# pppKin/rs_ray_toy

Hardware: AMD Instinct MI355X
Metric: Mrays/s (BVH ray queries, closest+any) @ 100k-tri heightfield 1024^2 256spp depth 8 (higher is better)
Workload: dtype f32; 1 GPU; BASELINE cfg4: procedural heightfield 100352 triangles, 1024x1024, 256 spp, Path max_depth 8, HaltonSampler, RealisticCamera, box filter; fixed-bvh BVH; film in interleaved 16-row bands, one gather to rank 0 per frame; 2 frame(s) in flight; collective=none (one rank), comm_world=1, triangles=100352, bvh_nodes=97951, bvh_depth=24

## Files before the change

### rs_ray_toy_amd/csrc/device/dkernels.hpp

```cpp
#pragma once
#include "dmath.hpp"
#include "dtexture.hpp"

namespace rrtd {

constexpr int kBlock = 256;
enum { C_ACTIVE = 0, C_NEXT = 32, C_SHADOW = 64, C_CAMERA_RAYS = 96, C_ERROR = 128, C_WORK_CLOSEST = 160, C_WORK_SHADOW = 192, C_WORK_AUX = 224, C_SHADOW2 = 256,
       C_WORK8_CLOSEST = 288, C_WORK8_SHADOW = 544,
       C_TT_DONE = 800,
       C_CULLED = 832,
       C_SKY = 864,
       C_RECORDS = 896, C_COUNT = 928 };
template <typename R> struct ShadeBlock { static constexpr int n = 256; };
#ifndef RRT_SHADE_BLOCK
#define RRT_SHADE_BLOCK 256
#endif
template <> struct ShadeBlock<float> { static constexpr int n = RRT_SHADE_BLOCK; };
enum { ERR_SHADING_NORMAL = 1, ERR_BETA = 4, ERR_NULL_BSDF = 8, ERR_MIPMAP = 16, ERR_HALTON_DIMS = 32, ERR_ST_DIMS = 64, ERR_NO_LIGHTS = 128,
       ERR_KIND_SET = 256  };
static_assert(ERR_ST_DIMS == kErrStDims, "error bit shared with dmath.hpp");
static_assert(ERR_HALTON_DIMS == kErrHaltonDims, "error bit shared with dmath.hpp");

template <typename R>
struct RayCtx {
// ... 850 lines not shown
#define RRT_SHADE_CHUNK 4u
#endif
#ifndef RRT_SHADE_WAVES
#define RRT_SHADE_WAVES 4
#endif
#ifndef RRT_SHADE_WAVES_LAMBERT
#define RRT_SHADE_WAVES_LAMBERT 6
#endif
#ifndef RRT_SHADE_BLOCK_LAMBERT
#define RRT_SHADE_BLOCK_LAMBERT 512
#endif
#ifndef RRT_SHADE_WAVES_GLOSSY
#define RRT_SHADE_WAVES_GLOSSY RRT_SHADE_WAVES
#endif
#ifndef RRT_SHADE_BLOCK_GLOSSY
#define RRT_SHADE_BLOCK_GLOSSY RRT_SHADE_BLOCK
#endif
template <typename R, uint32_t KM> constexpr int shade_path_block() {
  return sizeof(R) != 4 ? ShadeBlock<R>::n : (KM == kKindsLambert ? RRT_SHADE_BLOCK_LAMBERT : (KM == kKindsGlossy ? RRT_SHADE_BLOCK_GLOSSY : ShadeBlock<R>::n));
}
template <uint32_t KM> constexpr int shade_path_waves() { return KM == kKindsLambert ? RRT_SHADE_WAVES_LAMBERT : (KM == kKindsGlossy ? RRT_SHADE_WAVES_GLOSSY : RRT_SHADE_WAVES); }
template <typename R, int NL, bool TEX = false, uint32_t KM = kAllKinds, bool AREA = true>
__global__ void __launch_bounds__((shade_path_block<R, KM>())) __attribute__((amdgpu_waves_per_eu(TEX ? 1 : shade_path_waves<KM>(), 8))) k_shade_path(SceneDev<R> s, Pools<R> p) {
  __shared__ uint32_t push_lds[shade_path_block<R, KM>() / 64 + 1];
  constexpr uint32_t kShadeChunk = RRT_SHADE_CHUNK;
  __shared__ uint32_t hit_idx[kShadeChunk * shade_path_block<R, KM>()];
  const uint32_t n = p.counters[C_ACTIVE];
  using V4 = typename Vec4T<R>::type;
  const uint32_t chunk = s.shade_compact ? kShadeChunk : 1u;
  for (uint32_t base0 = blockIdx.x * blockDim.x * chunk; base0 < n; base0 += gridDim.x * blockDim.x * chunk) {
  uint32_t n_hits = min(blockDim.x, n - base0);
  if (chunk > 1u) {
    n_hits = 0u;
    for (uint32_t k = 0; k < chunk; k++) {
      const uint32_t e = base0 + k * blockDim.x + threadIdx.x;
      const bool is_hit = e < n && (int)real_to_bits(p.hit[e].y) >= 0;
      uint32_t cnt = 0;
      const uint32_t at = block_rank(is_hit, push_lds, &cnt);
      if (is_hit) hit_idx[n_hits + at] = e;
      n_hits += cnt;
    }
    __syncthreads();
  }
  for (uint32_t base = 0; base < n_hits; base += blockDim.x) {
  const uint32_t i = base + threadIdx.x < n_hits ? (chunk > 1u ? hit_idx[base + threadIdx.x] : base0 + base + threadIdx.x) : n;
  bool want_shadow = false, want_next = false, sky = false;
  uint32_t slot = 0;
  int prim = -1;
  V3<R> sh_o, sh_d, nx_o, nx_d, o_lo;
  Rgb<R> sh_ld, nx_beta;
  R nx_eta_scale = R(1);
  uint32_t index = 0, nx_db = 0, sh_tab = 0;
  if (i < n) {
    const QEnt qe = p.q_active[i];
    slot = qe.slot;
// ... 68 lines not shown
          if (cont && (int)bounces < s.max_depth && s.horizon != nullptr) {
            const float u = s.hz_axis == 0u ? (float)nd.x : (s.hz_axis == 1u ? (float)nd.y : (float)nd.z);
            const float a = s.hz_axis == 0u ? (float)nd.y : (s.hz_axis == 1u ? (float)nd.z : (float)nd.x), b = s.hz_axis == 0u ? (float)nd.z : (s.hz_axis == 1u ? (float)nd.x : (float)nd.y);
            const uint32_t q = s.horizon[(size_t)prim * 32u + (u < 0.0f ? 16u : 0u) + hz_sector(a, b)];
#ifdef RRT_HZ_NO_GUARD
            const float tau = -1.0f;
#else
            const float tau = s.hz_tau[prim];
#endif
            const bool above = fabsf(u) * 254.0f > (float)q;
            const bool inside = fminf(fminf((float)h.z, (float)h.w), 1.0f - (float)h.z - (float)h.w) * fabsf((float)dot(si.n, nd)) > tau;
            if (above && inside) { cont = false; sky = true; }
          }
          if (cont && (int)bounces < s.max_depth) {
            nx_o = si.p; nx_d = nd;
            nx_beta = beta; nx_eta_scale = eta_scale;
            nx_db = db_pack(s, dim, bounces);
            want_next = true;
          }
        }
      }
    }
  }
  const uint32_t qs = block_push(p.shadow_count, want_shadow, push_lds);
  if (want_shadow) {
    store_ray<R>(p.sray_o, p.sray_d, qs, sh_o, o_lo, sh_d, R(1) - R(0.0001), self_prim<R>(prim) | (int)(sh_tab << 24));
    p.sld[qs] = mk4u<R>(sh_ld.r, sh_ld.g, sh_ld.b, slot);
  }
  const uint32_t qn = block_push(&p.counters[C_NEXT], want_next, push_lds);
  if (want_next) {
    p.q_next[qn] = QEnt{slot, nx_db, index, 0u};
    p.npath[qn] = mk4<R>(nx_beta.r, nx_beta.g, nx_beta.b, nx_eta_scale);
    store_ray<R>(p.nray_o, p.nray_d, qn, nx_o, o_lo, nx_d, Const<R>::inf, self_prim<R>(prim));
  }
  if (s.horizon != nullptr) (void)block_push(&p.counters[C_SKY], sky, push_lds);
  }
  __syncthreads();
  }
}

template <typename R>
__global__ void __launch_bounds__(ShadeBlock<R>::n) k_shade_nee(SceneDev<R> s, Pools<R> p, int light_j, int first) {
  __shared__ uint32_t push_lds[ShadeBlock<R>::n / 64 + 1];
  using V4 = typename Vec4T<R>::type;
  const uint32_t i = blockIdx.x * blockDim.x + threadIdx.x;
  const uint32_t n = p.counters[C_ACTIVE];
  if (blockIdx.x * blockDim.x >= n) return;
  bool want_shadow = false;
  uint32_t slot = 0, sh_tab = 0;
  int prim = -1;
  V3<R> sh_o, sh_d, o_lo;
  Rgb<R> sh_ld;
  if (i < n) {
    const QEnt qe = p.q_active[i];
    slot = qe.slot;
    const V4 h = p.hit[i];
    prim = (int)real_to_bits(h.y);
    if (prim >= 0) {
// ... 223 lines not shown
          } else {
            R eta = R(1) / bsdf.eta;
            if (dot(wo, ns) < R(0)) { eta = R(1) / eta; ns = -ns; dndx = -dndx; dndy = -dndy; }
            const V3<R> dwodx = -fdr.rxd - wo, dwody = -fdr.ryd - wo;
            const R ddndx = dot(dwodx, ns) + dot(wo, dndx), ddndy = dot(dwody, ns) + dot(wo, dndy);
            const R mu = eta * dot(wo, ns) - absdot(wi, ns);
            const R dmudx = ddndx * (eta - (eta * eta * dot(wo, ns)) / absdot(wi, ns));
            const R dmudy = ddndy * (eta - (eta * eta * dot(wo, ns)) / absdot(wi, ns));
            cd.rxd = wi - dwodx * eta + (dndx * mu + ns * dmudx);
            cd.ryd = wi - dwody * eta + (dndy * mu + ns * dmudy);
          }
          c.dr = cd;
        }
      }
    }
  }
  V4 l = p.L[qe.slot];
  l.x += L.r; l.y += L.g; l.z += L.b;
  p.L[qe.slot] = l;
  if (n_closest) atomicAdd(&totals[2], (unsigned long long)n_closest);
  if (n_any) atomicAdd(&totals[3], (unsigned long long)n_any);
}

static __global__ void k_rotate(uint32_t* c, int what) {
  if (what == 0) { c[C_ACTIVE] = c[C_NEXT]; c[C_NEXT] = 0; c[C_SHADOW] = 0; }
  else if (what == 1) { c[C_SHADOW] = 0; }
  else if (what == 3) {  }
  else if (what == 4) { c[C_NEXT] = 0; }
  else if (what == 5) { c[C_ACTIVE] = c[C_NEXT]; c[C_NEXT] = 0; c[C_WORK_CLOSEST] = 0; c[C_WORK_AUX] = 0; for (int k = 0; k < 8; k++) c[C_WORK8_CLOSEST + 32 * k] = 0; return; }
  else if (what == 6) { c[C_SHADOW] = 0; c[C_WORK_SHADOW] = 0; for (int k = 0; k < 8; k++) c[C_WORK8_SHADOW + 32 * k] = 0; return; }
  else if (what == 7) { c[C_SHADOW2] = 0; c[C_WORK_SHADOW] = 0; for (int k = 0; k < 8; k++) c[C_WORK8_SHADOW + 32 * k] = 0; return; }
  else { c[C_ACTIVE] = 0; c[C_NEXT] = 0; c[C_SHADOW] = 0; c[C_RECORDS] = 0; }
  c[C_WORK_CLOSEST] = 0; c[C_WORK_SHADOW] = 0; c[C_WORK_AUX] = 0;
  for (int k = 0; k < 8; k++) { c[C_WORK8_CLOSEST + 32 * k] = 0; c[C_WORK8_SHADOW + 32 * k] = 0; }
}
static __global__ void k_accumulate_counts(uint32_t* c, unsigned long long* totals) {
  totals[2] += c[C_ACTIVE];
}
static __global__ void k_accumulate_shadow(const uint32_t* shadow_count, unsigned long long* totals) { totals[3] += *shadow_count; }
static __global__ void k_accumulate_sky(uint32_t* c, unsigned long long* totals) { totals[2] += c[C_SKY]; totals[8] += c[C_SKY]; c[C_SKY] = 0; }
static __global__ void k_accumulate_camera(uint32_t* c, unsigned long long* totals) {
  totals[4] += c[C_CAMERA_RAYS]; c[C_CAMERA_RAYS] = 0;
  totals[2] += c[C_CULLED]; totals[7] += c[C_CULLED]; c[C_CULLED] = 0;
}

template <typename R>
RRT_DEV Rgb<R> film_sample_radiance(const SceneDev<R>& s, R w, const typename Vec4T<R>::type& l) {
  Rgb<R> L;
  if (w > R(0)) L = Rgb<R>(l.x, l.y, l.z);
  if (L.has_nan()) L = Rgb<R>();
  else if (L.y() < R(-1e-5)) L = Rgb<R>();
  else if (isinf(L.y())) L = Rgb<R>();
  if (L.y() > s.max_sample_luminance) L = L * (s.max_sample_luminance / L.y());
  return L;
}
template <typename R>
RRT_DEV void film_box_add(const SceneDev<R>& s, R& cr, R& cg, R& cb, R& wsum, R w, const typename Vec4T<R>::type& l) {
  const Rgb<R> L = film_sample_radiance(s, w, l);
  cr += (L.r * w) * R(1); cg += (L.g * w) * R(1); cb += (L.b * w) * R(1);
  wsum += R(1);
}

template <typename R>
// ... 375 lines not shown
```

### rs_ray_toy_amd/csrc/device/dmath.hpp

```cpp
#pragma once
#include "dtypes.hpp"

namespace rrtd {

#define RRT_DEV __device__ __forceinline__

template <typename R> struct Const;
template <> struct Const<float> {
  static constexpr float one_minus_eps = 0.99999994f;
  static constexpr float machine_eps = 5.9604645e-8f;
  static constexpr float inf = __builtin_huge_valf();
};
template <> struct Const<double> {
  static constexpr double one_minus_eps = 0.99999999999999989;
  static constexpr double machine_eps = 1.1102230246251565e-16;
  static constexpr double inf = __builtin_huge_val();
};
#define RRT_PI 3.14159265358979323846
#define RRT_PI_OVER_2 1.57079632679489661923
#define RRT_PI_OVER_4 0.78539816339744830961

template <typename R> RRT_DEV R rsqrt_(R x) { return sqrt(x); }
RRT_DEV double rcp_r(double a) { return 1.0 / a; }
RRT_DEV float rcp_r(float a) { return __builtin_amdgcn_rcpf(a); }
// ... 103 lines not shown
  const uint32_t base = lds[nw] + lds[w];
  __syncthreads();
  return base + (uint32_t)__popcll(mask & ((1ull << lane) - 1ull));
}

RRT_DEV uint32_t block_push_range(uint32_t* counter, bool pred, uint32_t* lds, uint32_t* first, uint32_t* total) {
  const uint64_t mask = __ballot(pred);
  const uint32_t lane = __lane_id(), w = threadIdx.x >> 6, nw = (blockDim.x + 63u) >> 6;
  if (lane == 0) lds[w] = (uint32_t)__popcll(mask);
  __syncthreads();
  if (threadIdx.x == 0) {
    uint32_t tot = 0;
    for (uint32_t k = 0; k < nw; k++) { const uint32_t c = lds[k]; lds[k] = tot; tot += c; }
    lds[nw] = tot ? atomicAdd(counter, tot) : 0u;
    lds[nw + 1] = tot;
  }
  __syncthreads();
  *first = lds[nw]; *total = lds[nw + 1];
  const uint32_t base = lds[nw] + lds[w];
  __syncthreads();
  return base + (uint32_t)__popcll(mask & ((1ull << lane) - 1ull));
}

template <uint32_t... kOff>
RRT_DEV void block_push_multi(uint32_t* counters, uint32_t on, uint32_t pred, uint32_t* lds, uint32_t* at, uint32_t* first, uint32_t* total) {
  constexpr uint32_t kN = sizeof...(kOff);
  constexpr uint32_t off[kN] = {kOff...};
  const uint32_t lane = __lane_id(), w = threadIdx.x >> 6, nw = (blockDim.x + 63u) >> 6, stride = nw + 2u;
  uint64_t mask[kN];
#pragma unroll
  for (uint32_t i = 0; i < kN; i++) {
    mask[i] = __ballot((pred >> i) & 1u);
    if (lane == 0) lds[i * stride + w] = (uint32_t)__popcll(mask[i]);
  }
  __syncthreads();
  if (threadIdx.x < kN) {
    uint32_t o = off[0];
#pragma unroll
    for (uint32_t i = 1; i < kN; i++) if (threadIdx.x == i) o = off[i];
    uint32_t* l = lds + threadIdx.x * stride;
    uint32_t tot = 0;
    for (uint32_t k = 0; k < nw; k++) { const uint32_t n = l[k]; l[k] = tot; tot += n; }
    l[nw] = (tot && ((on >> threadIdx.x) & 1u)) ? atomicAdd(counters + o, tot) : 0u;
    l[nw + 1] = tot;
  }
  __syncthreads();
  const uint64_t below = (1ull << lane) - 1ull;
#pragma unroll
  for (uint32_t i = 0; i < kN; i++) {
    first[i] = lds[i * stride + nw]; total[i] = lds[i * stride + nw + 1];
    at[i] = first[i] + lds[i * stride + w] + (uint32_t)__popcll(mask[i] & below);
  }
  __syncthreads();
}

RRT_DEV uint32_t block_rank(bool pred, uint32_t* lds, uint32_t* total) {
  const uint64_t mask = __ballot(pred);
  const uint32_t lane = __lane_id(), w = threadIdx.x >> 6, nw = (blockDim.x + 63u) >> 6;
  if (lane == 0) lds[w] = (uint32_t)__popcll(mask);
  __syncthreads();
  if (threadIdx.x == 0) {
    uint32_t tot = 0;
    for (uint32_t k = 0; k < nw; k++) { const uint32_t c = lds[k]; lds[k] = tot; tot += c; }
    lds[nw] = tot;
  }
  __syncthreads();
  const uint32_t base = lds[w];
  *total = lds[nw];
  __syncthreads();
  return base + (uint32_t)__popcll(mask & ((1ull << lane) - 1ull));
}

RRT_DEV uint32_t div_base(uint32_t a, const HaltonDim& hd, uint32_t ) {
  const uint32_t t = __umulhi((uint32_t)hd.magic, a);
  return (t + ((a - t) >> 1)) >> (uint32_t)(hd.magic >> 32);
}
// ... 778 lines not shown
```

### rs_ray_toy_amd/csrc/device/dtraverse_f32.hpp

```cpp
#pragma once
#include "dkernels.hpp"
#include "lens_cull.hpp"

#ifndef RRT_VOTE_A
#define RRT_VOTE_A 1u
#define RRT_VOTE_B 2u
#endif
#ifndef RRT_NODE_STEPS
#define RRT_NODE_STEPS 2
#endif
#ifndef RRT_TR_REFILL
#define RRT_TR_REFILL 16u
#endif
namespace rrtd {

constexpr int kTravBlock = 512;
constexpr int kStackLds = 8;
constexpr int kTreeletNodes = 512;

struct alignas(64) PairNode {
  float xy0[4];
  float xy1[4];
  float zz[4];
  uint32_t id0, id1;
// ... 1151 lines not shown
        if (s.integrator != 0 ) p.path[qa] = make_float4(1.0f, 1.0f, 1.0f, 1.0f);
        p.ray_o[qa] = make_float4(wo.x, wo.y, wo.z, Const<float>::inf);
        p.ray_d[qa] = make_float4(wd.x, wd.y, wd.z, __uint_as_float(0xffffffffu));
      }
      if (!runs) { p.L[slot] = make_float4(0.0f, 0.0f, 0.0f, 0.0f); p.weight[slot] = w; }
      else if (rec) p.L[ref] = make_float4(0.0f, 0.0f, 0.0f, w);
    }
  }
}

RRT_DEV bool rg_trace_lean(const SceneDev<float>& s, const RgLensLds& lens, float pfx, float pfy, float lx, float ly, bool want_ray, RayT<float>& out) {
  RgLane L; L.phase = 0;
  const float w = rg_begin_lean(s, pfx, pfy, lx, ly, &L);
  bool ok = w != 0.0f;
  for (int k = s.n_lens - 1; k >= 0; k--) ok &= rg_step_lean(lens.a[k], lens.b[k], &L);
  if (ok && want_ray) {
    out.o = aff_pt(s.cam_m, V3<float>(L.o.x, L.o.y, -L.o.z));
    const V3<float> wdu = aff_vec(s.cam_m, V3<float>(L.d.x, L.d.y, -L.d.z));
    out.d = wdu * __builtin_amdgcn_rsqf(len2(wdu));
  }
  return ok;
}

static __global__ void __launch_bounds__(kRgDense) k_raygen_aux2_f32(SceneDev<float> s, Pools<float> p, int enqueue, int records) {
  __shared__ RgLensLds lens;
  __shared__ uint32_t push_lds[kRgDense / 64 + 1];
  const uint32_t tid = threadIdx.x;
  const uint32_t n = p.counters[C_NEXT];
  if (blockIdx.x * blockDim.x >= n) return;
  rg_lens_to_lds(s, &lens, tid);
  __syncthreads();
  const uint32_t i = blockIdx.x * blockDim.x + tid;
  const bool diffs = p.rdx_o != nullptr;
  bool alive = false;
  uint32_t slot = 0;
  float4 ro = make_float4(0, 0, 0, 0), rd = ro, cs = ro;
  if (i < n) {
    ro = p.nray_o[i]; rd = p.nray_d[i];
    slot = __float_as_uint(ro.w);
    cs = p.npath[i];
  }
  RayT<float> aux, auy;
  float epsx = 0.05f, epsy = 0.05f;
  bool okx = false, oky = false;
  for (int round = 0; round < 4; round++) {
    const bool is_x = (round & 1) == 0;
    const bool act = i < n && (round < 2 || (round == 2 ? !okx : (okx && !oky)));
    if (__ballot(act) == 0ull) continue;
    const float e = round < 2 ? 0.05f : -0.05f;
    RayT<float> out;
    bool ok = false;
    if (act) ok = rg_trace_lean(s, lens, cs.x + (is_x ? e : 0.0f), cs.y + (is_x ? 0.0f : e), cs.z, cs.w, diffs, out);
    if (act && is_x) { okx = ok; epsx = e; if (diffs) aux = out; }
    if (act && !is_x) { oky = ok; epsy = e; if (diffs) auy = out; }
  }
  alive = okx && oky;
  if (i < n) {
    if (alive && diffs) {
      const V3<float> o(ro.x, ro.y, ro.z), d(rd.x, rd.y, rd.z);
      V3<float> rxo = o + (aux.o - o) / epsx, rxd = d + (aux.d - d) / epsx;
      V3<float> ryo = o + (auy.o - o) / epsy, ryd = d + (auy.d - d) / epsy;
      rxo = o + (rxo - o) * s.diff_scale; ryo = o + (ryo - o) * s.diff_scale;
      rxd = d + (rxd - d) * s.diff_scale; ryd = d + (ryd - d) * s.diff_scale;
      p.rdx_o[slot] = make_float4(rxo.x, rxo.y, rxo.z, 0.0f); p.rdx_d[slot] = make_float4(rxd.x, rxd.y, rxd.z, 0.0f);
      p.rdy_o[slot] = make_float4(ryo.x, ryo.y, ryo.z, 0.0f); p.rdy_d[slot] = make_float4(ryd.x, ryd.y, ryd.z, 0.0f);
    }
  }
  const bool meets = !(s.root_cull && alive) || camera_ray_meets_root(s, V3<float>(ro.x, ro.y, ro.z), V3<float>(rd.x, rd.y, rd.z));
  const bool enq = alive && enqueue && meets;
  const uint32_t q = block_push(&p.counters[C_ACTIVE], enq, push_lds);
  if (s.root_cull) (void)block_push(&p.counters[C_CULLED], alive && enqueue && !meets, push_lds);
  (void)block_push(&p.counters[C_CAMERA_RAYS], alive, push_lds);
  if (enq) {
    p.q_active[q] = QEnt{slot, 5u, p.hindex[i], 0u};
    if (s.integrator != 0 ) p.path[q] = make_float4(1.0f, 1.0f, 1.0f, 1.0f);
    p.ray_o[q] = make_float4(ro.x, ro.y, ro.z, Const<float>::inf);
    p.ray_d[q] = make_float4(rd.x, rd.y, rd.z, __uint_as_float(0xffffffffu));
  }
  if (records) { if (i < n) p.L[slot] = make_float4(0.0f, 0.0f, 0.0f, alive ? rd.w : 0.0f); }
  else if (alive) { p.L[slot] = make_float4(0.0f, 0.0f, 0.0f, 0.0f); p.weight[slot] = rd.w; }
}

constexpr uint32_t kFrTiles = 4;
typedef float v4f __attribute__((ext_vector_type(4)));
static __global__ void __launch_bounds__(64 * kFrTiles) k_film_box_runs(SceneDev<float> s, Pools<float> p, PassDesc pd, float* film, const uint2* runs, uint32_t n_groups) {
  __shared__ v4f tab[kFrTiles][8][64];
  const uint32_t lane = threadIdx.x & 63u, wv = threadIdx.x >> 6;
  const uint32_t tile = blockIdx.x * kFrTiles + wv;
  const bool live = tile < pd.npix / 64u;
  const uint32_t* code = reinterpret_cast<const uint32_t*>(p.weight);
  float cr = 0.0f, cg = 0.0f, cb = 0.0f, wsum = 0.0f;
  float* px = film;
  if (live) {
    uint32_t x, y;
    pass_pixel(pd, pd.pix_begin + tile * 64u + lane, &x, &y);
    px = film + 4 * ((size_t)y * (uint32_t)s.xres + x);
    cr = px[0]; cg = px[1]; cb = px[2]; wsum = px[3];
  }
#pragma unroll
  for (uint32_t k = 0; k < 8; k++) tab[wv][k][lane] = v4f{0.0f, 0.0f, 0.0f, 0.0f};
  v4f rec[2][8];
  uint32_t cd[2][8];
  auto load = [&](auto B, uint32_t first, uint32_t cnt) {
// ... 41 lines not shown
```

### rs_ray_toy_amd/csrc/device/dtypes.hpp

```cpp
#pragma once
#include <hip/hip_runtime.h>
#include <stdint.h>

#include "horizon_build.hpp"
namespace rrtd {
struct HaltonBlk {
  uint32_t block;
  uint32_t shift;
  uint32_t magic;
  uint32_t lo_off, hi_off;
  uint32_t pad[3];
};

template <typename R>
struct alignas(sizeof(R) * 8) Node {
  R bmin[3];
  R bmax[3];
  uint32_t offset;
  uint32_t meta;
};

template <typename R>
struct alignas(16) Tri {
  R p0[3], p1[3], p2[3];
// ... 110 lines not shown
  uint32_t hz_axis;
  float root_box[6];
  const LensElem<R>* lens;
  int32_t n_lens, simple_weighting;
  R cam_m[12];
  R pupil0[4], pupil63[4];
  R shutter_open, shutter_close;
  int32_t xres, yres;
  R diagonal, extent[4];
  R max_sample_luminance;
  const R* filter_table;
  R filter_rx, filter_ry;
  R filter_inv_rx, filter_inv_ry;
  const HaltonDim* hdims;
  uint32_t* err;
  const uint16_t* perms;
  uint32_t nsamp, sample_at_center;
  uint32_t base_exp0, base_exp1, base_scale0, base_scale1, stride, mult_inv0, mult_inv1;
  uint32_t fast_div;
  uint32_t sampler_type;
  uint32_t st_nx, st_ny, st_jitter, st_dims, st_seed_lo, st_seed_hi;
  uint32_t cam_db;
  uint32_t shade_compact;
  uint32_t db_shift;
  uint32_t cam_perm[2];
  double cam_invpow[2][16];
  double cam_tail[2];
  double inv_base_scale1;
  double inv3pow[24];
  const uint32_t* cam_lo[3];
  const uint4* cam_hi[3];
  const HaltonBlk* hblk;
  const uint32_t* hlo;
  const uint4* hhi;
  uint32_t n_hblk;
  int32_t integrator, max_depth, light_strategy;
  R rr_threshold;
};

template <typename R> struct Vec4T;
template <> struct Vec4T<float> { using type = float4; };
template <> struct Vec4T<double> { using type = double4; };

struct alignas(16) QEnt { uint32_t slot, db, index, pad; };

template <typename R>
// ... 21 lines not shown
```

### rs_ray_toy_amd/csrc/device/rrt_impl.hpp

```cpp
#pragma once
#include <algorithm>
#include <atomic>
#include <chrono>
#include <cmath>
#include <cstdio>
#include <cstring>
#include <deque>
#include <mutex>
#include <memory>
#include <queue>
#include <stdexcept>
#include <string>
#include <thread>
#include <unordered_map>
#include <vector>

#include <type_traits>

#include "dfilter.hpp"
#include "dkernels.hpp"
#include "dtraverse_f32.hpp"
#include "rrt.h"

namespace rrtd {
// ... 498 lines not shown
  void gather_mark(bool begin) override {
    if (!pending_ || !frame_stats_) return;
    HIP_CHECK(hipSetDevice(dev_));
    hipEvent_t& e = ev_gather_[begin ? 0 : 1];
    if (!e) HIP_CHECK(hipEventCreate(&e));
    HIP_CHECK(hipEventRecord(e, st_));
    if (!begin) gather_marked_ = true;
  }
  void film_geometry(int* xres, int* yres, bool* splats) const override {
    const rrt_film& f = desc_.film;
    *xres = f.xres; *yres = f.yres;
    *splats = f.filter_type != RRT_FILTER_BOX || f.filter_radius[0] > 0.5 || f.filter_radius[1] > 0.5;
  }

  void set_option(const std::string& key, double v) override {
    if (key == "max_paths") { if (v < 64) throw std::invalid_argument("max_paths must be >= 64"); max_paths_ = (size_t)v; }
    else if (key == "count_traversal") count_traversal_ = v != 0;
    else if (key == "persistent_traversal") { persistent_ = v != 0; if (v >= 1) trav_mode_ = (int)v; }
    else if (key == "raygen_lean") raygen_lean_ = v != 0;
    else if (key == "tile_order") tile_order_ = v != 0;
    else if (key == "tile_trees") tile_trees_on_ = v != 0;
    else if (key == "quad_nodes") quad_on_ = v != 0;
    else if (key == "shade_compact") scene_.shade_compact = v != 0 ? 1u : 0u;
    else if (key == "horizon_cull") horizon_on_ = v != 0;
    else if (key == "root_cull") root_cull_on_ = v != 0;
    else if (key == "tt_census") { tt_census_spp_ = std::max(1, (int)v); tt_state_ = 0; }
    else if (key == "shadow_lists") shadow_lists_on_ = v != 0;
    else if (key == "sl_grid") sl_grid_cap_ = std::max(1, (int)v);
    else if (key == "rg_spb") {
      if (v != 1 && v != 2 && v != 4 && v != 8) throw std::invalid_argument("rg_spb must be 1, 2, 4 or 8");
      rg_spb_ = (int)v;
    }
    else if (key == "pt_split_closest") pt_split_closest_ = (uint32_t)v;
    else if (key == "pt_split_any") pt_split_any_ = (uint32_t)v;
    else if (key == "overlap_shadow") overlap_shadow_ = v != 0;
    else if (key == "aux_margin") aux_margin_ = v != 0;
    else if (key == "lens_cull") lens_cull_on_ = v != 0;
    else if (key == "film_records") film_records_on_ = v != 0;
    else if (key == "shade_spec") shade_kinds_ = v != 0 ? shade_kinds_scene_ : kAllKinds;
    else if (key == "frame_stats") frame_stats_ = v != 0;
    else if (key == "dn_lds") dn_lds_ = v != 0;
    else if (key == "halton_tables") scene_.n_hblk = (v != 0 && hblk_.n) ? (uint32_t)kHaltonTabDims : 0u;
    else if (key == "cam_tables") { for (int w = 0; w < 3; w++) { scene_.cam_lo[w] = (v != 0 && cam_lo_.n) ? cam_lo_.p + cam_lo_off_[w] : nullptr; scene_.cam_hi[w] = (v != 0 && cam_hi_.n) ? cam_hi_.p + cam_hi_off_[w] : nullptr; } }
    else if (key == "any_entry") { any_entry_on_ = v != 0; trav_.any_list = (any_entry_on_ && any_list_.n) ? reinterpret_cast<const uint4*>(any_list_.p) : nullptr; }
    else if (key == "nonblocking_streams") {
      if (pending_) throw std::invalid_argument("nonblocking_streams: a frame is in flight");
// ... 217 lines not shown
    };
    auto tock = [&](size_t id, hipStream_t stream = nullptr) { if (timing) HIP_CHECK(hipEventRecord(evs[id].second.second, stream ? stream : st_)); };
    uint64_t& n_closest_launch = fr->n_closest_launch;
    uint64_t& n_any_launch = fr->n_any_launch;
    const int integ = desc_.integrator.type;
    const int max_depth = desc_.integrator.max_depth;
    const size_t npix = pd.npix;
    const uint64_t ns = pd.ns;
    const size_t nslots = npix * (size_t)ns;
    const uint32_t grid = (uint32_t)((nslots + kBlock - 1) / kBlock);
    const uint32_t sgrid = (uint32_t)((nslots + ShadeBlock<R>::n - 1) / ShadeBlock<R>::n);
    hipLaunchKernelGGL(k_rotate, dim3(1), dim3(1), 0, st_, counters_.p, 2);
    size_t e = tick(0);
    launch_raygen(pd, grid, nullptr, integ != RRT_INT_AO ? 1 : 0, true, !with_moments, list);
    tock(e);
    hipLaunchKernelGGL(k_accumulate_camera, dim3(1), dim3(1), 0, st_, counters_.p, totals_.p);
    if (integ == RRT_INT_PATH) {
      const bool overlap = two_shadow_queues() && shadow_buf_[1][0] && !count_traversal_ && max_depth > 1;
      auto use_shadow_queue = [&](int k) {
        pool_.sray_o = shadow_buf_[k][0]; pool_.sray_d = shadow_buf_[k][1]; pool_.sld = shadow_buf_[k][2];
        pool_.shadow_count = counters_.p + (k ? C_SHADOW2 : C_SHADOW);
      };
      for (int b = 0; b < max_depth; b++) {
        hipLaunchKernelGGL(k_accumulate_counts, dim3(1), dim3(1), 0, st_, counters_.p, totals_.p);
        e = tick(1);
        launch_closest(nullptr, &counters_.p[C_ACTIVE], 0, count_traversal_, nullptr, nullptr, count_traversal_ ? totals_.p : nullptr, grid, b == 0);
        tock(e); n_closest_launch++;
        if (b == 0 && tt_pass_ok_ && !count_traversal_ && use_persistent()) fr->n_tile_launch++;
        if (overlap) {
          use_shadow_queue(b & 1);
          if (b > 1) HIP_CHECK(hipStreamWaitEvent(st_, ev_shadow_[b & 1], 0));
        }
        scene_.use_shadow_tabs = use_shadow_lists() ? 1u : 0u;
        scene_.horizon = (horizon_on_ && horizon_.n) ? horizon_.p : nullptr; scene_.hz_tau = horizon_tau_.p; scene_.hz_axis = hz_axis_;
        e = tick(3);
        if (tex_depth_ > 0) hipLaunchKernelGGL((k_shade_path<R, 4, true>), dim3(std::min((uint32_t)((nslots + 255) / 256), 16384u)), dim3(256), 0, st_, scene_, pool_);
        else if (has_translucent_) hipLaunchKernelGGL((k_shade_path<R, 4>), dim3(std::min((uint32_t)((nslots + 255) / 256), 16384u)), dim3(256), 0, st_, scene_, pool_);
        else if (shade_kinds_ == kKindsLambert) {
          constexpr uint32_t kB = (uint32_t)shade_path_block<R, kKindsLambert>();
          const dim3 g(std::min((uint32_t)((nslots + kB - 1) / kB), 16384u));
          if (area_lights_ || shade_kinds_ == kAllKinds) hipLaunchKernelGGL((k_shade_path<R, 2, false, kKindsLambert, true>), g, dim3(kB), 0, st_, scene_, pool_);
          else hipLaunchKernelGGL((k_shade_path<R, 2, false, kKindsLambert, false>), g, dim3(kB), 0, st_, scene_, pool_);
        }
        else if (shade_kinds_ == kKindsGlossy) {
          constexpr uint32_t kB = (uint32_t)shade_path_block<R, kKindsGlossy>();
          hipLaunchKernelGGL((k_shade_path<R, 2, false, kKindsGlossy>), dim3(std::min((uint32_t)((nslots + kB - 1) / kB), 16384u)), dim3(kB), 0, st_, scene_, pool_);
        }
        else hipLaunchKernelGGL((k_shade_path<R, 2>), dim3(std::min(sgrid, 16384u)), dim3(ShadeBlock<R>::n), 0, st_, scene_, pool_);
        tock(e);
        if (scene_.horizon) hipLaunchKernelGGL(k_accumulate_sky, dim3(1), dim3(1), 0, st_, counters_.p, totals_.p);
        if (overlap) {
          HIP_CHECK(hipEventRecord(ev_shade_, st_));
          HIP_CHECK(hipStreamWaitEvent(st2_, ev_shade_, 0));
          hipLaunchKernelGGL(k_accumulate_shadow, dim3(1), dim3(1), 0, st2_, pool_.shadow_count, totals_.p);
          e = tick(2, st2_);
          launch_shadow(grid, st2_);
          tock(e, st2_); n_any_launch++; if (use_shadow_lists()) fr->n_list_launch++;
          hipLaunchKernelGGL(k_rotate, dim3(1), dim3(1), 0, st2_, counters_.p, 6 + (b & 1));
          HIP_CHECK(hipEventRecord(ev_shadow_[b & 1], st2_));
          swap_queues();
          hipLaunchKernelGGL(k_rotate, dim3(1), dim3(1), 0, st_, counters_.p, 5);
        } else {
          hipLaunchKernelGGL(k_accumulate_shadow, dim3(1), dim3(1), 0, st_, pool_.shadow_count, totals_.p);
          e = tick(2);
          launch_shadow(grid);
          tock(e); n_any_launch++; if (use_shadow_lists()) fr->n_list_launch++;
          swap_queues();
          hipLaunchKernelGGL(k_rotate, dim3(1), dim3(1), 0, st_, counters_.p, 0);
        }
      }
      if (overlap) {
        HIP_CHECK(hipStreamWaitEvent(st_, ev_shadow_[(max_depth - 1) & 1], 0));
        use_shadow_queue(0);
      }
    } else if (integ == RRT_INT_DIRECT || integ == RRT_INT_DEBUG) {
      if (has_transmissive_ || tex_depth_ > 0) {
        size_t e2 = tick(3);
        TreeFrame<R>* deep = nullptr;
        if (max_depth > kTreeMax) {
          const size_t need = (size_t)(max_depth - kTreeMax) * nslots;
          if (tree_deep_.n < need) { HIP_CHECK(hipStreamSynchronize(st_)); tree_deep_.alloc(need); }
          deep = tree_deep_.p;
        }
        if (tex_depth_ > 0) hipLaunchKernelGGL((k_direct_tree<R, true>), dim3(grid), dim3(kBlock), 0, st_, scene_, pool_, totals_.p, deep, (uint32_t)nslots);
        else hipLaunchKernelGGL((k_direct_tree<R, false>), dim3(grid), dim3(kBlock), 0, st_, scene_, pool_, totals_.p, deep, (uint32_t)nslots);
        tock(e2);
      } else {
      const bool all = integ == RRT_INT_DEBUG || desc_.integrator.light_strategy == RRT_STRATEGY_ALL;
      for (int level = 0; level < std::max(1, max_depth - 1); level++) {
        hipLaunchKernelGGL(k_accumulate_counts, dim3(1), dim3(1), 0, st_, counters_.p, totals_.p);
        e = tick(1);
        launch_closest(nullptr, &counters_.p[C_ACTIVE], 0, count_traversal_, nullptr, nullptr, count_traversal_ ? totals_.p : nullptr, grid, level == 0);
        tock(e); n_closest_launch++;
        if (level == 0 && tt_pass_ok_ && !count_traversal_ && use_persistent()) fr->n_tile_launch++;
        if (desc_.n_lights > 0) {
          const int nl = all ? (int)desc_.n_lights : 1;
          for (int j = 0; j < nl; j++) {
            hipLaunchKernelGGL(k_rotate, dim3(1), dim3(1), 0, st_, counters_.p, 1);
            scene_.use_shadow_tabs = use_shadow_lists() ? 1u : 0u;
            e = tick(3);
            hipLaunchKernelGGL((k_shade_nee<R>), dim3(sgrid), dim3(ShadeBlock<R>::n), 0, st_, scene_, pool_, all ? j : -1, j == 0 ? 1 : 0);
            tock(e);
            hipLaunchKernelGGL(k_accumulate_shadow, dim3(1), dim3(1), 0, st_, pool_.shadow_count, totals_.p);
            e = tick(2);
            launch_shadow(grid);
            tock(e); n_any_launch++; if (use_shadow_lists()) fr->n_list_launch++;
          }
        }
        e = tick(3);
        hipLaunchKernelGGL((k_shade_specular<R>), dim3(sgrid), dim3(ShadeBlock<R>::n), 0, st_, scene_, pool_, (desc_.n_lights == 0 && integ == RRT_INT_DEBUG) ? 1 : 0);
        tock(e);
        swap_queues();
        hipLaunchKernelGGL(k_rotate, dim3(1), dim3(1), 0, st_, counters_.p, 0);
      }
      }
    }
    e = tick(4);
    if (!wide_filter && film_runs_ok_) {
      if constexpr (std::is_same<R, float>::value)
        hipLaunchKernelGGL(k_film_box_runs, dim3((uint32_t)((npix / 64 + kFrTiles - 1) / kFrTiles)), dim3(64 * kFrTiles), 0, st_, scene_, pool_, pd, film_.p, film_runs_.p, (uint32_t)(ns / 8));
    }
    else if (!wide_filter) {
      const dim3 fg((uint32_t)((npix + kBlock - 1) / kBlock));
      if (list) hipLaunchKernelGGL((k_film_box_moments_list<R>), fg, dim3(kBlock), 0, st_, scene_, pool_, pd, list, film_.p, moments_.p);
      else if (with_moments) hipLaunchKernelGGL((k_film_box_moments<R>), fg, dim3(kBlock), 0, st_, scene_, pool_, pd, film_.p, moments_.p);
      else hipLaunchKernelGGL((k_film_box<R>), fg, dim3(kBlock), 0, st_, scene_, pool_, pd, film_.p);
    }
    else {
      const int reach_x = (int)std::ceil(f.filter_radius[0] + 0.5), reach_y = (int)std::ceil(f.filter_radius[1] + 0.5);
      const int ex0 = std::max(0, rect[0] - reach_x), ey0 = std::max(0, rect[1] - reach_y);
      const int ex1 = std::min(f.xres, rect[2] + reach_x), ey1 = std::min(f.yres, rect[3] + reach_y);
      const size_t en = (size_t)(ex1 - ex0) * (size_t)(ey1 - ey0);
      const dim3 fg((uint32_t)((en + kBlock - 1) / kBlock));
      if (with_moments) hipLaunchKernelGGL((k_film_wide_moments<R>), fg, dim3(kBlock), 0, st_, scene_, pool_, pd, film_.p, moments_.p, ex0, ey0, ex1 - ex0, ey1 - ey0, reach_x, reach_y, f.yres);
      else hipLaunchKernelGGL((k_film_wide<R>), fg, dim3(kBlock), 0, st_, scene_, pool_, pd, film_.p, ex0, ey0, ex1 - ex0, ey1 - ey0, reach_x, reach_y, f.yres);
    }
// ... 861 lines not shown
          }
        }
        cam_lo_.upload(lo_all, st_); cam_hi_.upload(hi_all, st_);
        HIP_CHECK(hipStreamSynchronize(st_));
        for (int w = 0; w < 3; w++) { cam_lo_off_[w] = lo_off[w]; cam_hi_off_[w] = hi_off[w]; s.cam_lo[w] = cam_lo_.p + lo_off[w]; s.cam_hi[w] = cam_hi_.p + hi_off[w]; }
      }
    }
    {
      std::vector<R> ft(256);
      for (int i = 0; i < 256; i++) ft[i] = (R)d->film.filter_table[i];
      filter_table_.upload(ft, st_);
      HIP_CHECK(hipStreamSynchronize(st_));
      s.filter_table = filter_table_.p;
      s.filter_rx = (R)d->film.filter_radius[0]; s.filter_ry = (R)d->film.filter_radius[1];
      s.filter_inv_rx = (R)(1.0 / d->film.filter_radius[0]); s.filter_inv_ry = (R)(1.0 / d->film.filter_radius[1]);
    }
    s.sampler_type = (uint32_t)d->sampler.type;
    s.st_nx = (uint32_t)std::max(1, d->sampler.xsamp); s.st_ny = (uint32_t)std::max(1, d->sampler.ysamp);
    s.st_jitter = d->sampler.jitter ? 1u : 0u; s.st_dims = (uint32_t)std::max(0, d->sampler.dimension);
    s.st_seed_lo = (uint32_t)d->sampler.perm_seed; s.st_seed_hi = (uint32_t)(d->sampler.perm_seed >> 32);
    s.cam_db = d->sampler.type == RRT_SAMPLER_STRATIFIED ? (1u | (2u << kStBits)) : 5u;
    s.db_shift = d->sampler.type == RRT_SAMPLER_STRATIFIED ? kDbShiftStratified : kDbShiftHalton;
    s.shade_compact = 1u;
    s.integrator = d->integrator.type; s.max_depth = d->integrator.max_depth; s.light_strategy = d->integrator.light_strategy;
    s.rr_threshold = (R)d->integrator.rr_threshold;
    counters_.alloc(C_COUNT);
    HIP_CHECK(hipMemsetAsync(counters_.p, 0, C_COUNT * sizeof(uint32_t), st_));
    s.err = counters_.p + C_ERROR;
  }

  bool two_shadow_queues() const { return overlap_shadow_ && desc_.integrator.type == RRT_INT_PATH && !deep_; }
  size_t n_vec_records() const { return 12 + (tex_depth_ > 0 ? 4 : 0) + (two_shadow_queues() ? 3 : 0); }
  void ensure_pools(size_t n) {
    if (n <= cap_) return;
    HIP_CHECK(hipStreamSynchronize(st_));
    cap_ = n;
    using V4 = typename Vec4T<R>::type;
    const size_t NV = n_vec_records(), NR = 1, NU = 9;
    vpool_.alloc(NV * cap_);
    rpool_.alloc(NR * cap_);
    upool_.alloc(NU * cap_);
    Pools<R>& p = pool_;
    V4* v = vpool_.p;
    auto nv = [&]() { V4* x = v; v += cap_; return x; };
    p.ray_o = nv(); p.ray_d = nv(); p.nray_o = nv(); p.nray_d = nv(); p.hit = nv();
    p.sray_o = nv(); p.sray_d = nv(); p.sld = nv(); p.samp = nv(); p.path = nv(); p.npath = nv(); p.L = nv();
// ... 67 lines not shown
        const rrt_film& f = desc_.film;
        const int write_samp = (f.filter_type != RRT_FILTER_BOX || f.filter_radius[0] != 0.5 || f.filter_radius[1] != 0.5) ? 1 : 0;
        if (list) hipLaunchKernelGGL(k_pixel_offsets_list, dim3((pd.npix + kBlock - 1) / kBlock), dim3(kBlock), 0, st_, scene_, pool_, pd, list);
        else hipLaunchKernelGGL(k_pixel_offsets, dim3((pd.npix + kBlock - 1) / kBlock), dim3(kBlock), 0, st_, scene_, pool_, pd);
        {
          const float2* safe_r2 = (aux_margin_ && tex_depth_ == 0) ? reinterpret_cast<const float2*>(lens_safe_.p) : nullptr;
          const uint32_t* cull = (lens_cull_on_ && lens_cull_.n != 0 && tex_depth_ == 0 && pd.tiled) ? lens_cull_.p : nullptr;
          const uint32_t spb = (pd.tiled && pd.ns >= (uint32_t)rg_spb_) ? (uint32_t)std::max(1, std::min(rg_spb_, kRgDense / 64)) : 1u, ppb = kRgDense / spb;
          const uint32_t n_pb = (pd.npix + ppb - 1) / ppb, gz = (n_pb + 65534u) / 65535u, gy = (n_pb + gz - 1) / gz;
          if (!list && tt_state_ == 1 && tile_trees_on_ && enqueue && pd.tiled && spb == 8 && ppb == kTileW * kTileH && pd.pix_begin == 0 && pd.npix % ((uint32_t)pd.rw * kTileH) == 0 &&
              pd.ns % spb == 0 && use_persistent() && trav_mode_ == 3 && !count_traversal_) {
            const size_t n_chunks = (size_t)gy * gz * ((pd.ns + spb - 1) / spb);
            if (tt_chunks_.n < n_chunks) { HIP_CHECK(hipStreamSynchronize(st_)); tt_chunks_.alloc(n_chunks); }
            tt_pass_ = TileTrees{reinterpret_cast<const float4*>(tt_trees_.p), tt_tris_.p, tt_chunks_.p, (uint32_t)pd.rw / kTileW, pd.npix / (uint32_t)pd.rw / kTileH, pd.ns / spb, tt_mt_x_, tt_n_trees_, pd};
            tt_pass_ok_ = true;
            if (film_records_on_ && film_records && for_render && !dims_out && write_samp == 0 && tex_depth_ == 0 && desc_.integrator.type == RRT_INT_PATH) {
              if (film_runs_.n < n_chunks) { HIP_CHECK(hipStreamSynchronize(st_)); film_runs_.alloc(n_chunks); }
              film_runs_ok_ = true;
            }
          }
          hipLaunchKernelGGL(k_raygen_main_f32, dim3((pd.ns + spb - 1) / spb, gy, gz), dim3(kRgDense), 0, st_, scene_, pool_, pd, write_samp, dims_out, safe_r2, aux_delta_, aux_pupil_, enqueue, spb,
                             tt_pass_ok_ ? tt_chunks_.p : nullptr, cull, lc_inv_dr_, film_runs_ok_ ? film_runs_.p : nullptr);
          if (tt_pass_ok_) hipLaunchKernelGGL(k_tt_snapshot, dim3(1), dim3(1), 0, st_, counters_.p);
          hipLaunchKernelGGL(k_raygen_aux2_f32, dim3((total + kRgDense - 1) / kRgDense), dim3(kRgDense), 0, st_, scene_, pool_, enqueue, film_runs_ok_ ? 1 : 0);
          hipLaunchKernelGGL(k_rotate, dim3(1), dim3(1), 0, st_, counters_.p, 4);
        }
        HIP_CHECK(hipGetLastError());
        return;
      }
    }
    if (list) hipLaunchKernelGGL((k_raygen_list<R>), dim3(grid), dim3(kBlock), 0, st_, scene_, pool_, pd, list);
    else hipLaunchKernelGGL((k_raygen<R>), dim3(grid), dim3(kBlock), 0, st_, scene_, pool_, pd, dims_out);
    hipLaunchKernelGGL((k_raygen_aux<R>), dim3(grid), dim3(kBlock), 0, st_, scene_, pool_, enqueue);
    hipLaunchKernelGGL(k_rotate, dim3(1), dim3(1), 0, st_, counters_.p, 4);
    HIP_CHECK(hipGetLastError());
  }
  bool use_persistent() const { return std::is_same<R, float>::value && persistent_ && pairs_ok_; }
  void launch_persistent(bool any, const uint32_t* queue, const uint32_t* count, uint32_t n_fixed, uint32_t grid, uint8_t* occluded, hipStream_t stream = nullptr, bool tiles = false) {
    if constexpr (std::is_same<R, float>::value) {
      if (!stream) stream = st_;
      const uint32_t grid_in = grid;
      if (trav_grid_ == 0) {
        int per_cu = 0, cus = 0;
        HIP_CHECK(hipDeviceGetAttribute(&cus, hipDeviceAttributeMultiprocessorCount, dev_));
        if (mixed_) HIP_CHECK(hipOccupancyMaxActiveBlocksPerMultiprocessor(&per_cu, (k_trace_pairs_f32<false, true>), kTravBlock, 0));
        else HIP_CHECK(hipOccupancyMaxActiveBlocksPerMultiprocessor(&per_cu, (k_trace_pairs_f32<false, false>), kTravBlock, 0));
        trav_grid_ = (uint32_t)(std::max(1, per_cu) * std::max(1, cus));
// ... 543 lines not shown
```

Measured before the change: 7739 Mrays/s.

## Batch block-level queue pushes and fold per-bounce counter kernels

```diff
diff --git a/rs_ray_toy_amd/csrc/device/dkernels.hpp b/rs_ray_toy_amd/csrc/device/dkernels.hpp
--- a/rs_ray_toy_amd/csrc/device/dkernels.hpp
+++ b/rs_ray_toy_amd/csrc/device/dkernels.hpp
@@ -896,15 +896,27 @@
 template <uint32_t KM> constexpr int shade_path_waves() { return KM == kKindsLambert ? RRT_SHADE_WAVES_LAMBERT : (KM == kKindsGlossy ? RRT_SHADE_WAVES_GLOSSY : RRT_SHADE_WAVES); }
 template <typename R, int NL, bool TEX = false, uint32_t KM = kAllKinds, bool AREA = true>
 __global__ void __launch_bounds__((shade_path_block<R, KM>())) __attribute__((amdgpu_waves_per_eu(TEX ? 1 : shade_path_waves<KM>(), 8))) k_shade_path(SceneDev<R> s, Pools<R> p) {
-  __shared__ uint32_t push_lds[shade_path_block<R, KM>() / 64 + 1];
-  constexpr uint32_t kShadeChunk = RRT_SHADE_CHUNK;
+  constexpr uint32_t kShadeChunk = RRT_SHADE_CHUNK, kWaves = shade_path_block<R, KM>() / 64;
+  static_assert(kShadeChunk * kWaves <= 64u, "block_rank_multi: one wave prefixes the per-wave counts of a chunk");
+  __shared__ uint32_t push_lds[3 * (kWaves + 2) > kShadeChunk * kWaves + 1 ? 3 * (kWaves + 2) : kShadeChunk * kWaves + 1];
   __shared__ uint32_t hit_idx[kShadeChunk * shade_path_block<R, KM>()];
   const uint32_t n = p.counters[C_ACTIVE];
   using V4 = typename Vec4T<R>::type;
   const uint32_t chunk = s.shade_compact ? kShadeChunk : 1u;
   for (uint32_t base0 = blockIdx.x * blockDim.x * chunk; base0 < n; base0 += gridDim.x * blockDim.x * chunk) {
   uint32_t n_hits = min(blockDim.x, n - base0);
-  if (chunk > 1u) {
+  if (chunk > 1u && s.shade_push_multi) {
+    uint32_t hits = 0u, rank[kShadeChunk];
+#pragma unroll
+    for (uint32_t k = 0; k < kShadeChunk; k++) {
+      const uint32_t e = base0 + k * blockDim.x + threadIdx.x;
+      hits |= (e < n && (int)real_to_bits(p.hit[e].y) >= 0 ? 1u : 0u) << k;
+    }
+    n_hits = block_rank_multi<kShadeChunk>(hits, push_lds, rank);
+#pragma unroll
+    for (uint32_t k = 0; k < kShadeChunk; k++) if ((hits >> k) & 1u) hit_idx[rank[k]] = base0 + k * blockDim.x + threadIdx.x;
+    __syncthreads();
+  } else if (chunk > 1u) {
     n_hits = 0u;
     for (uint32_t k = 0; k < chunk; k++) {
       const uint32_t e = base0 + k * blockDim.x + threadIdx.x;
@@ -1019,18 +1031,24 @@
       }
     }
   }
-  const uint32_t qs = block_push(p.shadow_count, want_shadow, push_lds);
+  uint32_t qs, qn = 0u;
+  if (s.shade_push_multi) {
+    uint32_t at[3], first[3], total[3];
+    block_push_multi_at<4u>(s.horizon != nullptr ? 7u : 3u, (want_shadow ? 1u : 0u) | (want_next ? 2u : 0u) | (sky ? 4u : 0u), push_lds, at, first, total,
+                            p.shadow_count, &p.counters[C_NEXT], &p.counters[C_SKY]);
+    qs = at[0]; qn = at[1];
+  } else qs = block_push(p.shadow_count, want_shadow, push_lds);
   if (want_shadow) {
     store_ray<R>(p.sray_o, p.sray_d, qs, sh_o, o_lo, sh_d, R(1) - R(0.0001), self_prim<R>(prim) | (int)(sh_tab << 24));
     p.sld[qs] = mk4u<R>(sh_ld.r, sh_ld.g, sh_ld.b, slot);
   }
-  const uint32_t qn = block_push(&p.counters[C_NEXT], want_next, push_lds);
+  if (!s.shade_push_multi) qn = block_push(&p.counters[C_NEXT], want_next, push_lds);
   if (want_next) {
     p.q_next[qn] = QEnt{slot, nx_db, index, 0u};
     p.npath[qn] = mk4<R>(nx_beta.r, nx_beta.g, nx_beta.b, nx_eta_scale);
     store_ray<R>(p.nray_o, p.nray_d, qn, nx_o, o_lo, nx_d, Const<R>::inf, self_prim<R>(prim));
   }
-  if (s.horizon != nullptr) (void)block_push(&p.counters[C_SKY], sky, push_lds);
+  if (!s.shade_push_multi && s.horizon != nullptr) (void)block_push(&p.counters[C_SKY], sky, push_lds);
   }
   __syncthreads();
   }
@@ -1300,7 +1318,7 @@
   if (n_any) atomicAdd(&totals[3], (unsigned long long)n_any);
 }
 
-static __global__ void k_rotate(uint32_t* c, int what) {
+RRT_DEV void rotate_counters(uint32_t* c, int what) {
   if (what == 0) { c[C_ACTIVE] = c[C_NEXT]; c[C_NEXT] = 0; c[C_SHADOW] = 0; }
   else if (what == 1) { c[C_SHADOW] = 0; }
   else if (what == 3) {  }
@@ -1312,11 +1330,16 @@
   c[C_WORK_CLOSEST] = 0; c[C_WORK_SHADOW] = 0; c[C_WORK_AUX] = 0;
   for (int k = 0; k < 8; k++) { c[C_WORK8_CLOSEST + 32 * k] = 0; c[C_WORK8_SHADOW + 32 * k] = 0; }
 }
+static __global__ void k_rotate(uint32_t* c, int what) { rotate_counters(c, what); }
+static __global__ void k_bounce_end(uint32_t* c, unsigned long long* totals, int what, int sky, int count_next) {
+  if (sky) { totals[2] += c[C_SKY]; totals[8] += c[C_SKY]; c[C_SKY] = 0; }
+  rotate_counters(c, what);
+  if (count_next) totals[2] += c[C_ACTIVE];
+}
 static __global__ void k_accumulate_counts(uint32_t* c, unsigned long long* totals) {
   totals[2] += c[C_ACTIVE];
 }
 static __global__ void k_accumulate_shadow(const uint32_t* shadow_count, unsigned long long* totals) { totals[3] += *shadow_count; }
-static __global__ void k_accumulate_sky(uint32_t* c, unsigned long long* totals) { totals[2] += c[C_SKY]; totals[8] += c[C_SKY]; c[C_SKY] = 0; }
 static __global__ void k_accumulate_camera(uint32_t* c, unsigned long long* totals) {
   totals[4] += c[C_CAMERA_RAYS]; c[C_CAMERA_RAYS] = 0;
   totals[2] += c[C_CULLED]; totals[7] += c[C_CULLED]; c[C_CULLED] = 0;
diff --git a/rs_ray_toy_amd/csrc/device/dmath.hpp b/rs_ray_toy_amd/csrc/device/dmath.hpp
--- a/rs_ray_toy_amd/csrc/device/dmath.hpp
+++ b/rs_ray_toy_amd/csrc/device/dmath.hpp
@@ -149,10 +149,9 @@
   return base + (uint32_t)__popcll(mask & ((1ull << lane) - 1ull));
 }
 
-template <uint32_t... kOff>
-RRT_DEV void block_push_multi(uint32_t* counters, uint32_t on, uint32_t pred, uint32_t* lds, uint32_t* at, uint32_t* first, uint32_t* total) {
-  constexpr uint32_t kN = sizeof...(kOff);
-  constexpr uint32_t off[kN] = {kOff...};
+template <uint32_t kCountOnly = 0u, typename... C>
+RRT_DEV void block_push_multi_at(uint32_t on, uint32_t pred, uint32_t* lds, uint32_t* at, uint32_t* first, uint32_t* total, C*... ctr) {
+  constexpr uint32_t kN = sizeof...(C);
   const uint32_t lane = __lane_id(), w = threadIdx.x >> 6, nw = (blockDim.x + 63u) >> 6, stride = nw + 2u;
   uint64_t mask[kN];
 #pragma unroll
@@ -162,23 +161,54 @@
   }
   __syncthreads();
   if (threadIdx.x < kN) {
-    uint32_t o = off[0];
-#pragma unroll
-    for (uint32_t i = 1; i < kN; i++) if (threadIdx.x == i) o = off[i];
+    uint32_t* c = nullptr;
+    uint32_t i = 0;
+    ((c = threadIdx.x == i++ ? ctr : c), ...);
     uint32_t* l = lds + threadIdx.x * stride;
     uint32_t tot = 0;
     for (uint32_t k = 0; k < nw; k++) { const uint32_t n = l[k]; l[k] = tot; tot += n; }
-    l[nw] = (tot && ((on >> threadIdx.x) & 1u)) ? atomicAdd(counters + o, tot) : 0u;
+    l[nw] = (tot && ((on >> threadIdx.x) & 1u)) ? atomicAdd(c, tot) : 0u;
     l[nw + 1] = tot;
   }
   __syncthreads();
   const uint64_t below = (1ull << lane) - 1ull;
 #pragma unroll
   for (uint32_t i = 0; i < kN; i++) {
-    first[i] = lds[i * stride + nw]; total[i] = lds[i * stride + nw + 1];
+    total[i] = lds[i * stride + nw + 1];
+    if ((kCountOnly >> i) & 1u) { first[i] = 0u; at[i] = 0u; continue; }
+    first[i] = lds[i * stride + nw];
     at[i] = first[i] + lds[i * stride + w] + (uint32_t)__popcll(mask[i] & below);
   }
   __syncthreads();
+}
+template <uint32_t... kOff>
+RRT_DEV void block_push_multi(uint32_t* counters, uint32_t on, uint32_t pred, uint32_t* lds, uint32_t* at, uint32_t* first, uint32_t* total) {
+  block_push_multi_at(on, pred, lds, at, first, total, (counters + kOff)...);
+}
+
+template <uint32_t kK>
+RRT_DEV uint32_t block_rank_multi(uint32_t pred, uint32_t* lds, uint32_t* rank) {
+  const uint32_t lane = __lane_id(), w = threadIdx.x >> 6, nw = (blockDim.x + 63u) >> 6;
+  uint64_t mask[kK];
+#pragma unroll
+  for (uint32_t k = 0; k < kK; k++) {
+    mask[k] = __ballot((pred >> k) & 1u);
+    if (lane == 0) lds[k * nw + w] = (uint32_t)__popcll(mask[k]);
+  }
+  __syncthreads();
+  if (w == 0) {
+    const uint32_t cnt = lane < kK * nw ? lds[lane] : 0u;
+    uint32_t incl = cnt;
+#pragma unroll
+    for (uint32_t d = 1; d < 64u; d <<= 1) { const uint32_t up = __shfl_up(incl, d); if (lane >= d) incl += up; }
+    if (lane < kK * nw) lds[lane] = incl - cnt;
+    if (lane == 63u) lds[kK * nw] = incl;
+  }
+  __syncthreads();
+  const uint64_t below = (1ull << lane) - 1ull;
+#pragma unroll
+  for (uint32_t k = 0; k < kK; k++) rank[k] = lds[k * nw + w] + (uint32_t)__popcll(mask[k] & below);
+  return lds[kK * nw];
 }
 
 RRT_DEV uint32_t block_rank(bool pred, uint32_t* lds, uint32_t* total) {
diff --git a/rs_ray_toy_amd/csrc/device/dtraverse_f32.hpp b/rs_ray_toy_amd/csrc/device/dtraverse_f32.hpp
--- a/rs_ray_toy_amd/csrc/device/dtraverse_f32.hpp
+++ b/rs_ray_toy_amd/csrc/device/dtraverse_f32.hpp
@@ -1197,16 +1197,18 @@
   return ok;
 }
 
+constexpr uint32_t kRgAuxGrid = 2048;
 static __global__ void __launch_bounds__(kRgDense) k_raygen_aux2_f32(SceneDev<float> s, Pools<float> p, int enqueue, int records) {
   __shared__ RgLensLds lens;
-  __shared__ uint32_t push_lds[kRgDense / 64 + 1];
+  __shared__ uint32_t push_lds[3 * (kRgDense / 64 + 2)];
   const uint32_t tid = threadIdx.x;
   const uint32_t n = p.counters[C_NEXT];
   if (blockIdx.x * blockDim.x >= n) return;
   rg_lens_to_lds(s, &lens, tid);
   __syncthreads();
-  const uint32_t i = blockIdx.x * blockDim.x + tid;
   const bool diffs = p.rdx_o != nullptr;
+  for (uint32_t base = blockIdx.x * blockDim.x; base < n; base += gridDim.x * blockDim.x) {
+  const uint32_t i = base + tid;
   bool alive = false;
   uint32_t slot = 0;
   float4 ro = make_float4(0, 0, 0, 0), rd = ro, cs = ro;
@@ -1243,9 +1245,10 @@
   }
   const bool meets = !(s.root_cull && alive) || camera_ray_meets_root(s, V3<float>(ro.x, ro.y, ro.z), V3<float>(rd.x, rd.y, rd.z));
   const bool enq = alive && enqueue && meets;
-  const uint32_t q = block_push(&p.counters[C_ACTIVE], enq, push_lds);
-  if (s.root_cull) (void)block_push(&p.counters[C_CULLED], alive && enqueue && !meets, push_lds);
-  (void)block_push(&p.counters[C_CAMERA_RAYS], alive, push_lds);
+  uint32_t at[3], first[3], total[3];
+  block_push_multi_at<6u>(s.root_cull ? 7u : 5u, (enq ? 1u : 0u) | (alive && enqueue && !meets ? 2u : 0u) | (alive ? 4u : 0u), push_lds, at, first, total,
+                          &p.counters[C_ACTIVE], &p.counters[C_CULLED], &p.counters[C_CAMERA_RAYS]);
+  const uint32_t q = at[0];
   if (enq) {
     p.q_active[q] = QEnt{slot, 5u, p.hindex[i], 0u};
     if (s.integrator != 0 ) p.path[q] = make_float4(1.0f, 1.0f, 1.0f, 1.0f);
@@ -1254,6 +1257,7 @@
   }
   if (records) { if (i < n) p.L[slot] = make_float4(0.0f, 0.0f, 0.0f, alive ? rd.w : 0.0f); }
   else if (alive) { p.L[slot] = make_float4(0.0f, 0.0f, 0.0f, 0.0f); p.weight[slot] = rd.w; }
+  }
 }
 
 constexpr uint32_t kFrTiles = 4;
diff --git a/rs_ray_toy_amd/csrc/device/dtypes.hpp b/rs_ray_toy_amd/csrc/device/dtypes.hpp
--- a/rs_ray_toy_amd/csrc/device/dtypes.hpp
+++ b/rs_ray_toy_amd/csrc/device/dtypes.hpp
@@ -156,6 +156,7 @@
   uint32_t st_nx, st_ny, st_jitter, st_dims, st_seed_lo, st_seed_hi;
   uint32_t cam_db;
   uint32_t shade_compact;
+  uint32_t shade_push_multi;
   uint32_t db_shift;
   uint32_t cam_perm[2];
   double cam_invpow[2][16];
diff --git a/rs_ray_toy_amd/csrc/device/rrt_impl.hpp b/rs_ray_toy_amd/csrc/device/rrt_impl.hpp
--- a/rs_ray_toy_amd/csrc/device/rrt_impl.hpp
+++ b/rs_ray_toy_amd/csrc/device/rrt_impl.hpp
@@ -544,6 +544,7 @@
     else if (key == "tile_trees") tile_trees_on_ = v != 0;
     else if (key == "quad_nodes") quad_on_ = v != 0;
     else if (key == "shade_compact") scene_.shade_compact = v != 0 ? 1u : 0u;
+    else if (key == "shade_push_multi") scene_.shade_push_multi = v != 0 ? 1u : 0u;
     else if (key == "horizon_cull") horizon_on_ = v != 0;
     else if (key == "root_cull") root_cull_on_ = v != 0;
     else if (key == "tt_census") { tt_census_spp_ = std::max(1, (int)v); tt_state_ = 0; }
@@ -807,7 +808,7 @@
         pool_.shadow_count = counters_.p + (k ? C_SHADOW2 : C_SHADOW);
       };
       for (int b = 0; b < max_depth; b++) {
-        hipLaunchKernelGGL(k_accumulate_counts, dim3(1), dim3(1), 0, st_, counters_.p, totals_.p);
+        if (b == 0) hipLaunchKernelGGL(k_accumulate_counts, dim3(1), dim3(1), 0, st_, counters_.p, totals_.p);
         e = tick(1);
         launch_closest(nullptr, &counters_.p[C_ACTIVE], 0, count_traversal_, nullptr, nullptr, count_traversal_ ? totals_.p : nullptr, grid, b == 0);
         tock(e); n_closest_launch++;
@@ -833,7 +834,7 @@
         }
         else hipLaunchKernelGGL((k_shade_path<R, 2>), dim3(std::min(sgrid, 16384u)), dim3(ShadeBlock<R>::n), 0, st_, scene_, pool_);
         tock(e);
-        if (scene_.horizon) hipLaunchKernelGGL(k_accumulate_sky, dim3(1), dim3(1), 0, st_, counters_.p, totals_.p);
+        const int sky = scene_.horizon ? 1 : 0, count_next = b + 1 < max_depth ? 1 : 0;
         if (overlap) {
           HIP_CHECK(hipEventRecord(ev_shade_, st_));
           HIP_CHECK(hipStreamWaitEvent(st2_, ev_shade_, 0));
@@ -844,14 +845,14 @@
           hipLaunchKernelGGL(k_rotate, dim3(1), dim3(1), 0, st2_, counters_.p, 6 + (b & 1));
           HIP_CHECK(hipEventRecord(ev_shadow_[b & 1], st2_));
           swap_queues();
-          hipLaunchKernelGGL(k_rotate, dim3(1), dim3(1), 0, st_, counters_.p, 5);
+          hipLaunchKernelGGL(k_bounce_end, dim3(1), dim3(1), 0, st_, counters_.p, totals_.p, 5, sky, count_next);
         } else {
           hipLaunchKernelGGL(k_accumulate_shadow, dim3(1), dim3(1), 0, st_, pool_.shadow_count, totals_.p);
           e = tick(2);
           launch_shadow(grid);
           tock(e); n_any_launch++; if (use_shadow_lists()) fr->n_list_launch++;
           swap_queues();
-          hipLaunchKernelGGL(k_rotate, dim3(1), dim3(1), 0, st_, counters_.p, 0);
+          hipLaunchKernelGGL(k_bounce_end, dim3(1), dim3(1), 0, st_, counters_.p, totals_.p, 0, sky, count_next);
         }
       }
       if (overlap) {
@@ -872,8 +873,9 @@
         tock(e2);
       } else {
       const bool all = integ == RRT_INT_DEBUG || desc_.integrator.light_strategy == RRT_STRATEGY_ALL;
-      for (int level = 0; level < std::max(1, max_depth - 1); level++) {
-        hipLaunchKernelGGL(k_accumulate_counts, dim3(1), dim3(1), 0, st_, counters_.p, totals_.p);
+      const int n_levels = std::max(1, max_depth - 1);
+      for (int level = 0; level < n_levels; level++) {
+        if (level == 0) hipLaunchKernelGGL(k_accumulate_counts, dim3(1), dim3(1), 0, st_, counters_.p, totals_.p);
         e = tick(1);
         launch_closest(nullptr, &counters_.p[C_ACTIVE], 0, count_traversal_, nullptr, nullptr, count_traversal_ ? totals_.p : nullptr, grid, level == 0);
         tock(e); n_closest_launch++;
@@ -896,7 +898,7 @@
         hipLaunchKernelGGL((k_shade_specular<R>), dim3(sgrid), dim3(ShadeBlock<R>::n), 0, st_, scene_, pool_, (desc_.n_lights == 0 && integ == RRT_INT_DEBUG) ? 1 : 0);
         tock(e);
         swap_queues();
-        hipLaunchKernelGGL(k_rotate, dim3(1), dim3(1), 0, st_, counters_.p, 0);
+        hipLaunchKernelGGL(k_bounce_end, dim3(1), dim3(1), 0, st_, counters_.p, totals_.p, 0, 0, level + 1 < n_levels ? 1 : 0);
       }
       }
     }
@@ -1804,6 +1806,7 @@
     s.cam_db = d->sampler.type == RRT_SAMPLER_STRATIFIED ? (1u | (2u << kStBits)) : 5u;
     s.db_shift = d->sampler.type == RRT_SAMPLER_STRATIFIED ? kDbShiftStratified : kDbShiftHalton;
     s.shade_compact = 1u;
+    s.shade_push_multi = 1u;
     s.integrator = d->integrator.type; s.max_depth = d->integrator.max_depth; s.light_strategy = d->integrator.light_strategy;
     s.rr_threshold = (R)d->integrator.rr_threshold;
     counters_.alloc(C_COUNT);
@@ -1917,7 +1920,7 @@
           hipLaunchKernelGGL(k_raygen_main_f32, dim3((pd.ns + spb - 1) / spb, gy, gz), dim3(kRgDense), 0, st_, scene_, pool_, pd, write_samp, dims_out, safe_r2, aux_delta_, aux_pupil_, enqueue, spb,
                              tt_pass_ok_ ? tt_chunks_.p : nullptr, cull, lc_inv_dr_, film_runs_ok_ ? film_runs_.p : nullptr);
           if (tt_pass_ok_) hipLaunchKernelGGL(k_tt_snapshot, dim3(1), dim3(1), 0, st_, counters_.p);
-          hipLaunchKernelGGL(k_raygen_aux2_f32, dim3((total + kRgDense - 1) / kRgDense), dim3(kRgDense), 0, st_, scene_, pool_, enqueue, film_runs_ok_ ? 1 : 0);
+          hipLaunchKernelGGL(k_raygen_aux2_f32, dim3(std::min((total + kRgDense - 1) / kRgDense, kRgAuxGrid)), dim3(kRgDense), 0, st_, scene_, pool_, enqueue, film_runs_ok_ ? 1 : 0);
           hipLaunchKernelGGL(k_rotate, dim3(1), dim3(1), 0, st_, counters_.p, 4);
         }
         HIP_CHECK(hipGetLastError());
```

Result: no change. 7765 Mrays/s, median of 4 (+0.3%).
